# stefanch/sGDML

Measured on AMD Instinct MI355X. Metric: kernel-matrix build+solve wall-clock, N_train=1000 21-atom (aspirin-sized), lower is better.
Workload: dtype f64

## Files before the change

### include/gdml_hip.h

```cpp
#ifndef GDML_HIP_H
#define GDML_HIP_H

#include <stdint.h>

#ifdef __cplusplus
extern "C" {
#endif

typedef struct gdml_ctx gdml_ctx;

typedef enum {
  GDML_OK = 0,
  GDML_ERR_INVALID = -1,
  GDML_ERR_HIP = -2,
  GDML_ERR_OOM = -3,
  GDML_ERR_STATE = -4,
  GDML_ERR_NOT_PD = -5,
  GDML_ERR_UNSUPPORTED = -6,
  GDML_ERR_COMM = -7
} gdml_status;


int gdml_abi_version(void);

// ... 36 lines not shown
                    int64_t col_b, const int64_t* idx, int64_t n_idx, int64_t alloc_extra_rows,
                    double* K_host_out, int64_t ldk);

int gdml_assemble_A(gdml_ctx* ctx, double sig, double lam, int use_E_cstr, int64_t alloc_extra_rows);

int gdml_K_shape(gdml_ctx* ctx, int64_t* n_rows, int64_t* n_cols, int64_t* extra_rows);

int gdml_chol_set_rhs(gdml_ctx* ctx, const double* y, int64_t n);
int gdml_lu_solve(gdml_ctx* ctx, double lam, const double* y, int64_t n, double* alphas_out, int* info);
int gdml_chol_factor(gdml_ctx* ctx, double lam, int* info);
int gdml_chol_solve(gdml_ctx* ctx, const double* y, int64_t n, int n_refine, double* alphas_out);

int gdml_predict_upload_model(gdml_ctx* ctx, const double* R_desc, const double* R_d_desc_alpha,
                              int64_t M, int N, const int64_t* tril_perms, int P, double sig,
                              const double* alphas_E);
int gdml_set_alphas(gdml_ctx* ctx, const double* alphas_F, const double* alphas_E);
int gdml_predict(gdml_ctx* ctx, const double* R, int64_t B, const double* lat,
                 const double* lat_inv, double* E_out, double* F_out);

int gdml_predict_dev(gdml_ctx* ctx, const double* R_dev, int64_t B, const double* lat,
                     const double* lat_inv, double* E_dev, double* F_dev);

int gdml_predict_hessian(gdml_ctx* ctx, const double* R, int64_t B, const double* lat, const double* lat_inv,
                         double* E_out, double* F_out, double* H_out);
int gdml_predict_hessian_dev(gdml_ctx* ctx, const double* R_dev, int64_t B, const double* lat,
                             const double* lat_inv, double* E_dev, double* F_dev, double* H_dev);

int gdml_uncert_prepare(gdml_ctx* ctx, double sig, double lam, int* info);
int gdml_uncert_release(gdml_ctx* ctx);
int gdml_uncert_cross(gdml_ctx* ctx, const double* R, int64_t B, const double* lat, const double* lat_inv,
                      double* Kx_out, double* kqq_out);
int gdml_predict_cov(gdml_ctx* ctx, const double* R, int64_t B, const double* lat, const double* lat_inv, int full,
                     double* cov_out);
int gdml_predict_cov_dev(gdml_ctx* ctx, const double* R_dev, int64_t B, const double* lat, const double* lat_inv,
                         int full, double* cov_dev);

int gdml_loo(gdml_ctx* ctx, const double* alphas, int64_t n, int cov_mode, double* resid_out, double* cov_out,
             double* logdet_out, int* info);

int gdml_factor_extend(gdml_ctx* ctx, const double* R_desc_new, const double* R_d_desc_new, int64_t b, int* info);

int gdml_factor_remove(gdml_ctx* ctx, const int64_t* idx, int64_t b, int* info);

int gdml_predict_errors(gdml_ctx* ctx, const double* R, int64_t B, const double* lat,
                        const double* lat_inv, double std, double c, const double* E_ref,
                        const double* F_ref, double* sums8_out);

int gdml_kernel_matvec(gdml_ctx* ctx, double lam, int use_E_cstr, const double* v, int64_t n,
                       double* out);

typedef int (*gdml_pcg_cb)(int64_t iter, double resid, void* user);
int gdml_nystroem_factor(gdml_ctx* ctx, double lam, const int64_t* idx, int64_t m,
                         double* lev_scores_out, double* LinvKmn_host_out, int* info);
int gdml_nystroem_lev_scores(gdml_ctx* ctx, double* lev_scores_out);
int gdml_precon_apply(gdml_ctx* ctx, double lam, const double* v, int64_t n, double* out);
int gdml_pcg(gdml_ctx* ctx, double lam, int use_E_cstr, const double* y, const double* x0,
             int64_t n, double rtol, int64_t maxiter, int use_precon, gdml_pcg_cb cb,
             int64_t cb_every, void* user, double* x_out, int64_t* iters_out, double* resid_out,
             int* info_out);
int gdml_pcg_x(gdml_ctx* ctx, double* x_host_out);

int gdml_comm_unique_id(void* id128_out);
int gdml_comm_init(gdml_ctx* ctx, const void* id128, int rank, int world);
int gdml_comm_info(gdml_ctx* ctx, int* rank_out, int* world_out);
int gdml_comm_suspend(gdml_ctx* ctx, int suspend);

int gdml_dist_chol_solve(gdml_ctx* ctx, double sig, double lam, const double* y, int64_t n, double* alphas_out,
                         int* info);

typedef int (*gdml_host_allreduce)(double* buf, int64_t count, void* user);
typedef int (*gdml_host_allgather)(double* buf, int64_t chunk, void* user);
int gdml_comm_init_host(gdml_ctx* ctx, int rank, int world, gdml_host_allreduce allreduce,
                        gdml_host_allgather allgather, void* user);

int gdml_comm_stats(gdml_ctx* ctx, int64_t* calls_out, double* bytes_out);

int gdml_dev_alloc(gdml_ctx* ctx, int64_t bytes, void** dev_out);
int gdml_dev_free(gdml_ctx* ctx, void* dev);
int gdml_memcpy_h2d(gdml_ctx* ctx, void* dev, const void* host, int64_t bytes);
int gdml_memcpy_d2h(gdml_ctx* ctx, void* host, const void* dev, int64_t bytes);

int gdml_K_dev(gdml_ctx* ctx, double** K_dev_out, int64_t* ld_out);

#ifdef __cplusplus
}
#endif
#endif
```

### sgdml_amd/_lib.py

```python
import ctypes as C
import os

import numpy as np

_HERE = os.path.dirname(os.path.abspath(__file__))
LIB_PATH = os.environ.get('GDML_HIP_LIB', os.path.join(_HERE, 'libgdml_hip.so'))

GDML_OK = 0
ERR_INVALID, ERR_HIP, ERR_OOM, ERR_STATE, ERR_NOT_PD, ERR_UNSUPPORTED, ERR_COMM = -1, -2, -3, -4, -5, -6, -7
COLS_ALL, COLS_POINTS, COLS_INDEX = 0, 1, 2

_dp = C.POINTER(C.c_double)
_ip = C.POINTER(C.c_int64)
_vp = C.c_void_p
PCG_CB = C.CFUNCTYPE(C.c_int, C.c_int64, C.c_double, _vp)
HOST_COLL_CB = C.CFUNCTYPE(C.c_int, _dp, C.c_int64, _vp)

SIGNATURES = {
    'gdml_abi_version': (C.c_int, []),
    'gdml_device_count': (C.c_int, [C.POINTER(C.c_int)]),
    'gdml_device_pci_bus_id': (C.c_int, [C.c_int, C.c_char_p, C.c_int]),
    'gdml_ctx_create': (C.c_int, [C.c_int, C.POINTER(_vp)]),
    'gdml_ctx_destroy': (C.c_int, [_vp]),
    'gdml_last_error': (C.c_char_p, [_vp]),
    'gdml_sync': (C.c_int, [_vp]),
    'gdml_mem_info': (C.c_int, [_vp, _ip, _ip, _ip]),
    'gdml_mem_reserve': (C.c_int, [_vp, C.c_int64, _ip]),
    'gdml_phase_ms': (C.c_int, [_vp, C.c_char_p, _dp, _ip]),
    'gdml_profile': (C.c_int, [_vp, C.c_int]),
    'gdml_kernel_stat': (C.c_int, [_vp, C.c_char_p, _dp, _ip, _dp]),
    'gdml_desc_from_R': (C.c_int, [_vp, _vp, C.c_int64, C.c_int, _vp, _vp, _vp, _vp]),
    'gdml_sym_eig_absv': (C.c_int, [_vp, _vp, C.c_int64, C.c_int, _vp]),
    'gdml_perm_match': (C.c_int, [_vp, _vp, _vp, _vp, C.c_int64, C.c_int, _vp, _vp, _vp, C.c_int64, C.POINTER(C.c_int64)]),
    'gdml_train_upload': (C.c_int, [_vp, _vp, _vp, C.c_int64, C.c_int, _vp, C.c_int]),
    'gdml_assemble_K': (C.c_int, [_vp, C.c_double, C.c_int, C.c_int, C.c_int64, C.c_int64, _vp, C.c_int64,
                                  C.c_int64, _vp, C.c_int64]),
    'gdml_assemble_A': (C.c_int, [_vp, C.c_double, C.c_double, C.c_int, C.c_int64]),
    'gdml_K_shape': (C.c_int, [_vp, _ip, _ip, _ip]),
    'gdml_chol_set_rhs': (C.c_int, [_vp, _vp, C.c_int64]),
    'gdml_chol_factor': (C.c_int, [_vp, C.c_double, C.POINTER(C.c_int)]),
    'gdml_lu_solve': (C.c_int, [_vp, C.c_double, _vp, C.c_int64, _vp, C.POINTER(C.c_int)]),
    'gdml_chol_solve': (C.c_int, [_vp, _vp, C.c_int64, C.c_int, _vp]),
    'gdml_predict_upload_model': (C.c_int, [_vp, _vp, _vp, C.c_int64, C.c_int, _vp, C.c_int, C.c_double, _vp]),
    'gdml_set_alphas': (C.c_int, [_vp, _vp, _vp]),
    'gdml_predict': (C.c_int, [_vp, _vp, C.c_int64, _vp, _vp, _vp, _vp]),
    'gdml_predict_dev': (C.c_int, [_vp, _vp, C.c_int64, _vp, _vp, _vp, _vp]),
    'gdml_predict_hessian': (C.c_int, [_vp, _vp, C.c_int64, _vp, _vp, _vp, _vp, _vp]),
    'gdml_predict_hessian_dev': (C.c_int, [_vp, _vp, C.c_int64, _vp, _vp, _vp, _vp, _vp]),
    'gdml_uncert_prepare': (C.c_int, [_vp, C.c_double, C.c_double, C.POINTER(C.c_int)]),
    'gdml_uncert_release': (C.c_int, [_vp]),
    'gdml_uncert_cross': (C.c_int, [_vp, _vp, C.c_int64, _vp, _vp, _vp, _vp]),
    'gdml_predict_cov': (C.c_int, [_vp, _vp, C.c_int64, _vp, _vp, C.c_int, _vp]),
    'gdml_predict_cov_dev': (C.c_int, [_vp, _vp, C.c_int64, _vp, _vp, C.c_int, _vp]),
    'gdml_loo': (C.c_int, [_vp, _vp, C.c_int64, C.c_int, _vp, _vp, C.POINTER(C.c_double), C.POINTER(C.c_int)]),
    'gdml_factor_extend': (C.c_int, [_vp, _vp, _vp, C.c_int64, C.POINTER(C.c_int)]),
    'gdml_factor_remove': (C.c_int, [_vp, _vp, C.c_int64, C.POINTER(C.c_int)]),
    'gdml_kernel_matvec': (C.c_int, [_vp, C.c_double, C.c_int, _vp, C.c_int64, _vp]),
    'gdml_predict_errors': (C.c_int, [_vp, _vp, C.c_int64, _vp, _vp, C.c_double, C.c_double, _vp, _vp, _vp]),
    'gdml_nystroem_factor': (C.c_int, [_vp, C.c_double, _vp, C.c_int64, _vp, _vp, C.POINTER(C.c_int)]),
    'gdml_nystroem_lev_scores': (C.c_int, [_vp, _vp]),
    'gdml_precon_apply': (C.c_int, [_vp, C.c_double, _vp, C.c_int64, _vp]),
    'gdml_pcg': (C.c_int, [_vp, C.c_double, C.c_int, _vp, _vp, C.c_int64, C.c_double, C.c_int64, C.c_int,
                           PCG_CB, C.c_int64, _vp, _vp, _ip, _dp, C.POINTER(C.c_int)]),
    'gdml_pcg_x': (C.c_int, [_vp, _vp]),
    'gdml_dist_chol_solve': (C.c_int, [_vp, C.c_double, C.c_double, _vp, C.c_int64, _vp, C.POINTER(C.c_int)]),
    'gdml_comm_unique_id': (C.c_int, [_vp]),
    'gdml_comm_init': (C.c_int, [_vp, _vp, C.c_int, C.c_int]),
    'gdml_comm_info': (C.c_int, [_vp, C.POINTER(C.c_int), C.POINTER(C.c_int)]),
    'gdml_comm_suspend': (C.c_int, [_vp, C.c_int]),
    'gdml_comm_init_host': (C.c_int, [_vp, C.c_int, C.c_int, HOST_COLL_CB, HOST_COLL_CB, _vp]),
    'gdml_comm_stats': (C.c_int, [_vp, _ip, _dp]),
    'gdml_set_option': (C.c_int, [_vp, C.c_char_p, C.c_double]),
    'gdml_get_option': (C.c_int, [_vp, C.c_char_p, _dp, C.POINTER(C.c_int)]),
    'gdml_dev_alloc': (C.c_int, [_vp, C.c_int64, C.POINTER(_vp)]),
    'gdml_dev_free': (C.c_int, [_vp, _vp]),
    'gdml_memcpy_h2d': (C.c_int, [_vp, _vp, _vp, C.c_int64]),
    'gdml_memcpy_d2h': (C.c_int, [_vp, _vp, _vp, C.c_int64]),
    'gdml_K_dev': (C.c_int, [_vp, C.POINTER(_vp), _ip]),
}

_lib = None


class GDMLHipError(RuntimeError):
    pass


def load():
    global _lib
    if _lib is not None:
        return _lib
    if not os.path.exists(LIB_PATH):
        raise ImportError(
            'libgdml_hip.so not found at {} -- build it with `python -c "import __graft_entry__ as g; '
            'g.build()"` or `make -C sgdml_amd/csrc`. There is no CPU fallback.'.format(LIB_PATH)
        )
    lib = C.CDLL(LIB_PATH)
    for name, (res, args) in SIGNATURES.items():
        fn = getattr(lib, name)
        fn.restype = res
        fn.argtypes = args
    _lib = lib
    return lib


def device_count():
    n = C.c_int(0)
    load().gdml_device_count(C.byref(n))
    return n.value


def device_pci_bus_id(device):
    buf = C.create_string_buffer(64)
    if load().gdml_device_pci_bus_id(int(device), buf, 64) != 0:
        return None
    return buf.value.decode() or None


def preflight(attempts=3, timeout=180):
    import subprocess
    import sys

    if device_count() < 1:
        return 0
    code = ('import numpy as np; from sgdml_amd import _lib; c = _lib.Context(0); '
            'c.desc_from_R(np.arange(18.0).reshape(2, 9) ** 1.5, 3); c.close()')
    root = os.path.dirname(os.path.dirname(os.path.abspath(__file__)))
    err = ''
    for k in range(1, attempts + 1):
        try:
            p = subprocess.run([sys.executable, '-c', code], cwd=root, capture_output=True, text=True, timeout=timeout)
            if p.returncode == 0:
                return k
            err = (p.stderr or '')[-400:]
        except subprocess.TimeoutExpired:
            err = 'timeout'
    raise RuntimeError('GPU preflight failed %d times: %s' % (attempts, err))


def _ptr(a):
    return None if a is None else a.ctypes.data_as(_vp)


def f64(a):
    return None if a is None else np.ascontiguousarray(a, dtype=np.float64)


def i64(a):
    return None if a is None else np.ascontiguousarray(a, dtype=np.int64)


def _digest(a):
    try:
        import xxhash

        return xxhash.xxh64(memoryview(a).cast('B')).hexdigest()
    except ImportError:
        import hashlib

        return hashlib.md5(memoryview(a).cast('B')).hexdigest()

# ... 519 lines not shown
```

### sgdml_amd/csrc/chol.hip

```cpp
#include "common.h"
#include <type_traits>
#include <utility>

typedef double d4 __attribute__((ext_vector_type(4)));
typedef double d2 __attribute__((ext_vector_type(2)));

#define GT 128
#define GBK 16
#define GPITCH 17

struct GemmArgs {
  const double* A;
  const double* B;
  double* C;
  int64_t M, N, K, lda, ldb, ldc;
  int lower;
  int tiles_m, tiles_n;
  int64_t n_super;
  int64_t s_begin;
  int super_n;
  int aligned;
  int cyc_W, cyc_rank;
  int64_t cyc_lb0, cyc_nb, cyc_col0, cyc_block_rows;
  double* diagA;
  int diag_nbw;
  int64_t diag_off;
  int* diag_info;
  int col0_first;
  int* ready;
  int ready_target, ready_rows;
  const double* A2;
  const double* B2;
  double* C2;
  int64_t M2, N2, K2;
  int tiles2;
};

__global__ void __launch_bounds__(256, 2) gemm_nt_sub_diag_kernel(GemmArgs g);

template <bool FULL>
__device__ __forceinline__ void gemm_load_tile(const double* __restrict__ G, int64_t ld,
                                               int64_t row0, int64_t nrows, int64_t k0, int64_t K,
                                               int tid, d2 (&r)[4]) {
#pragma unroll
  for (int s = 0; s < 4; ++s) {
    int cidx = tid + 256 * s;
    int row = cidx >> 3, kc = (cidx & 7) * 2;
    int64_t gr = row0 + row, gk = k0 + kc;
    if (FULL) {
      r[s] = *reinterpret_cast<const d2*>(G + gr * ld + gk);
    } else {
      int64_t cr = gr < nrows ? gr : nrows - 1;
      int64_t ck0 = gk < K ? gk : K - 1, ck1 = gk + 1 < K ? gk + 1 : K - 1;
      double v0 = G[cr * ld + ck0], v1 = G[cr * ld + ck1];
      d2 v;
      v.x = (gr < nrows && gk < K) ? v0 : 0.0;
      v.y = (gr < nrows && gk + 1 < K) ? v1 : 0.0;
      r[s] = v;
    }
  }
}

__device__ __forceinline__ void gemm_load_tile_g(const double* __restrict__ base, const unsigned (&off)[4], d2 (&r)[4]) {
  typedef const __attribute__((address_space(1))) char* gcptr;
  typedef const __attribute__((address_space(1))) d2* gd2ptr;
  const uint64_t p = reinterpret_cast<uint64_t>(base);
  const uint32_t lo = __builtin_amdgcn_readfirstlane((uint32_t)p), hi = __builtin_amdgcn_readfirstlane((uint32_t)(p >> 32));
  gcptr b = (gcptr)(((uint64_t)hi << 32) | lo);
#pragma unroll
  for (int s = 0; s < 4; ++s) r[s] = *(gd2ptr)(b + off[s]);
}

__device__ __forceinline__ void gemm_store_tile16(double* __restrict__ S, int tid, const d2 (&r)[4]) {
  d2* S2 = reinterpret_cast<d2*>(S);
#pragma unroll
  for (int s = 0; s < 4; ++s) {
    const int cidx = tid + 256 * s;
    const int row = cidx >> 3, kq = cidx & 7;
    S2[kq * 128 + (row ^ kq)] = r[s];
  }
}

template <bool FULL, bool OW>
__device__ __forceinline__ void gemm_tile_body(const GemmArgs& g, double (*lds)[2][GT * GPITCH], int64_t row0, int64_t col0) {
  const int tid = threadIdx.x, lane = tid & 63, wave = tid >> 6;
  const int wm = wave >> 1, wn = wave & 1;
  const int li = lane & 15, lk = lane >> 4;

  const int wu = __builtin_amdgcn_readfirstlane(wave);
  double* const Ct = g.C + (row0 + (wu >> 1) * 64) * g.ldc + col0 + (wu & 1) * 64;
  const unsigned coff = (unsigned)lk * (unsigned)g.ldc + (unsigned)li;
  d4 acc[4][4];
#pragma unroll
  for (int i = 0; i < 4; ++i)
#pragma unroll
    for (int j = 0; j < 4; ++j) {
      if (FULL && !OW) {
#pragma unroll
        for (int r = 0; r < 4; ++r) acc[i][j][r] = -(Ct + (int64_t)(i * 16 + 4 * r) * g.ldc)[coff + j * 16];
      } else {
        acc[i][j] = (d4){0.0, 0.0, 0.0, 0.0};
      }
    }

  const int nk32 = (int)((g.K + GBK - 1) / GBK);
  d2 ra[4], rb[4];
  gemm_load_tile<FULL>(g.A, g.lda, row0, g.M, 0, g.K, tid, ra);
  gemm_load_tile<FULL>(g.B, g.ldb, col0, g.N, 0, g.K, tid, rb);
  gemm_store_tile16(lds[0][0], tid, ra);
  gemm_store_tile16(lds[0][1], tid, rb);
  __syncthreads();

  const int c16 = lane & 15, gq = lane >> 4;
  unsigned offA[4], offB[4];
#pragma unroll
  for (int s4 = 0; s4 < 4; ++s4) {
    const int cidx = tid + 256 * s4;
    offA[s4] = (unsigned)(((int64_t)(cidx >> 3) * g.lda + (cidx & 7) * 2) * 8);
    offB[s4] = (unsigned)(((int64_t)(cidx >> 3) * g.ldb + (cidx & 7) * 2) * 8);
  }
  const double* const Abase = g.A + row0 * g.lda;
// ... 52 lines not shown
  };
  for (int kt = 0; kt + 1 < nk32; ++kt) step(kt, std::true_type{});
  step(nk32 - 1, std::false_type{});

  if (FULL) {
    double* Ct2g = Ct;
    unsigned coff2 = coff;
    asm volatile("" : "+v"(Ct2g), "+v"(coff2));
    __attribute__((address_space(1))) double* Ct2 = (__attribute__((address_space(1))) double*)Ct2g;
#pragma unroll
    for (int j = 0; j < 4; ++j)
#pragma unroll
      for (int i = 0; i < 4; ++i)
#pragma unroll
        for (int r = 0; r < 4; ++r) (Ct2 + (int64_t)(i * 16 + 4 * r) * g.ldc)[coff2 + j * 16] = -acc[i][j][r];
    return;
  }
  if constexpr (OW) {
#pragma unroll
    for (int j = 0; j < 4; ++j) {
      const int64_t gc = col0 + wn * 64 + j * 16 + li;
#pragma unroll
      for (int i = 0; i < 4; ++i)
#pragma unroll
        for (int r = 0; r < 4; ++r) {
          const int64_t gr = row0 + wm * 64 + i * 16 + lk + 4 * r;
          if (gc < g.N && gr < g.M) g.C[gr * g.ldc + gc] = -acc[i][j][r];
        }
    }
    return;
  }
#pragma unroll
  for (int j = 0; j < 4; ++j) {
    double cv[4][4];
    const int64_t gc = col0 + wn * 64 + j * 16 + li;
    const bool cok = gc < g.N;
#pragma unroll
    for (int i = 0; i < 4; ++i)
#pragma unroll
      for (int r = 0; r < 4; ++r) {
        const int64_t gr = row0 + wm * 64 + i * 16 + lk + 4 * r;
        const int64_t cr = gr < g.M ? gr : g.M - 1, cc = cok ? gc : g.N - 1;
        cv[i][r] = g.C[cr * g.ldc + cc];
      }
#pragma unroll
    for (int i = 0; i < 4; ++i)
#pragma unroll
      for (int r = 0; r < 4; ++r) {
        const int64_t gr = row0 + wm * 64 + i * 16 + lk + 4 * r;
        if (cok && gr < g.M) g.C[gr * g.ldc + gc] = cv[i][r] - acc[i][j][r];
      }
  }
}

template <bool OW>
__device__ __forceinline__ void gemm_block(const GemmArgs& g, double (*lds)[2][GT * GPITCH], int64_t b) {
  if (b < g.tiles2) {
    const int tn2 = (int)((g.N2 + GT - 1) / GT);
    const int64_t ti = b / tn2, tj = b - ti * tn2;
    if (ti < tn2 && tj > ti) return;
    GemmArgs h = g;
    h.A = g.A2; h.B = g.B2; h.C = g.C2; h.M = g.M2; h.N = g.N2; h.K = g.K2;
    h.aligned = ((reinterpret_cast<uintptr_t>(g.A2) | reinterpret_cast<uintptr_t>(g.B2)) & 15) == 0 && g.aligned;
    const int64_t row0 = ti * GT, col0 = tj * GT;
    const bool full = (row0 + GT <= h.M) && (col0 + GT <= h.N) && ((h.K & (GBK - 1)) == 0) && h.aligned;
    if (full)
      gemm_tile_body<true, false>(h, lds, row0, col0);
    else
      gemm_tile_body<false, false>(h, lds, row0, col0);
    if (g.ready && ti < g.ready_rows && tj < g.ready_rows) {
      __threadfence();
      __syncthreads();
      if (threadIdx.x == 0) atomicAdd(g.ready, 1);
    }
    return;
  }
  b -= g.tiles2;
  const int64_t xcd = b & 7, loc = b >> 3;
  const int64_t s = g.s_begin + (loc >> 6) * 8 + xcd;
  const int within = (int)(loc & 63);
  if (s >= g.n_super) return;
  int64_t SI, SJ;
  if (g.lower) {
    int64_t sr = s, shift = 0;
    const int64_t sm = (g.tiles_m + 7) / 8;
    if (g.col0_first) {
      if (s < sm) { SI = s; SJ = 0; sr = -1; }
      else { sr = s - sm; shift = 1; }
    }
    if (sr >= 0) {
      SI = (int64_t)((sqrt(8.0 * (double)sr + 1.0) - 1.0) * 0.5);
      while (SI * (SI + 1) / 2 > sr) --SI;
      while ((SI + 1) * (SI + 2) / 2 <= sr) ++SI;
      SJ = sr - SI * (SI + 1) / 2;
      SI += shift; SJ += shift;
    }
  } else {
    SI = s / g.super_n;
    SJ = s - SI * g.super_n;
  }
  const int64_t ti = SI * 8 + (within >> 3), tj = SJ * 8 + (within & 7);
  if (ti >= g.tiles_m || tj >= g.tiles_n) return;
  if (g.lower && tj > ti) return;
  const int64_t row0 = ti * GT, col0 = tj * GT;
  if (g.cyc_W > 0 && row0 + GT <= g.cyc_block_rows) {
    const int64_t gb = (g.cyc_lb0 + row0 / g.cyc_nb) * g.cyc_W + g.cyc_rank;
    const int64_t grow_last = gb * g.cyc_nb + (row0 + GT - 1) % g.cyc_nb;
    if (g.cyc_col0 + col0 > grow_last) return;
  }
  const bool full = (row0 + GT <= g.M) && (col0 + GT <= g.N) && ((g.K & (GBK - 1)) == 0) && g.aligned;
  if (full)
    gemm_tile_body<true, OW>(g, lds, row0, col0);
  else
    gemm_tile_body<false, OW>(g, lds, row0, col0);
  if (g.ready && g.tiles2 == 0 && ti < g.ready_rows && tj < g.ready_rows) {
    __threadfence();
    __syncthreads();
    if (threadIdx.x == 0) atomicAdd(g.ready, 1);
  }
}

__global__ void __launch_bounds__(256, 2) gemm_nt_sub_kernel(GemmArgs g) {
  __shared__ __attribute__((aligned(16))) double lds[2][2][GT * GPITCH];
  gemm_block<false>(g, lds, blockIdx.x);
}


__global__ void __launch_bounds__(256, 2) gemm_nt_neg_kernel(GemmArgs g) {
  __shared__ __attribute__((aligned(16))) double lds[2][2][GT * GPITCH];
  gemm_block<true>(g, lds, blockIdx.x);
}

struct DiagJob {
  double* A = nullptr;
  int nbw = 0;
  int64_t off = 0;
  int* ready = nullptr;
  int ready_target = 0;
  bool col0_first = false;
  const double* A2 = nullptr;
  const double* B2 = nullptr;
  double* C2 = nullptr;
  int64_t M2 = 0, N2 = 0, K2 = 0;
};

static int launch_gemm_nt_sub_part(gdml_ctx* ctx, hipStream_t st, const double* A, int64_t lda,
                                   const double* B, int64_t ldb, double* C, int64_t ldc, int64_t M,
                                   int64_t N, int64_t K, int lower, double f0, double f1, bool timed,
                                   const DiagJob* diag = nullptr, const CyclicLower* cyc = nullptr, bool overwrite = false) {
  if (M <= 0 || N <= 0 || K <= 0) return GDML_OK;
  GemmArgs g;
  g.A = A; g.B = B; g.C = C; g.M = M; g.N = N; g.K = K; g.lda = lda; g.ldb = ldb; g.ldc = ldc;
  g.lower = lower;
  g.diagA = nullptr; g.diag_nbw = 0; g.diag_off = 0; g.diag_info = nullptr;
  g.cyc_W = 0; g.cyc_rank = 0; g.cyc_lb0 = 0; g.cyc_nb = 0; g.cyc_col0 = 0; g.cyc_block_rows = 0;
  g.col0_first = (diag && diag->col0_first) ? 1 : 0;
  g.ready = nullptr; g.ready_target = 0; g.ready_rows = 0;
  g.A2 = g.B2 = nullptr; g.C2 = nullptr; g.M2 = g.N2 = g.K2 = 0; g.tiles2 = 0;
  if (cyc) { g.cyc_W = cyc->W; g.cyc_rank = cyc->rank; g.cyc_lb0 = cyc->lb0; g.cyc_nb = cyc->nb; g.cyc_col0 = cyc->col0; g.cyc_block_rows = cyc->block_rows; }
  g.aligned = ((reinterpret_cast<uintptr_t>(A) | reinterpret_cast<uintptr_t>(B)) & 15) == 0 &&
              (lda % 2 == 0) && (ldb % 2 == 0);
  g.tiles_m = (int)((M + GT - 1) / GT);
  g.tiles_n = (int)((N + GT - 1) / GT);
  int64_t sm = (g.tiles_m + 7) / 8, sn = (g.tiles_n + 7) / 8;
  g.super_n = (int)sn;
  const int64_t n_super_all = lower ? sm * (sm + 1) / 2 : sm * sn;
  g.s_begin = (int64_t)(f0 * (double)n_super_all);
  g.n_super = (f1 >= 1.0) ? n_super_all : (int64_t)(f1 * (double)n_super_all);
  const bool has_diag = diag && diag->A;
  if (g.n_super <= g.s_begin) {
    if (!has_diag) return GDML_OK;
    g.n_super = g.s_begin;
  }
  int64_t groups = (g.n_super - g.s_begin + 7) / 8;
  int64_t blocks = groups * 512;
  const int slot = (timed && st == (ctx->kt_stream ? ctx->kt_stream : ctx->stream)) ? ktime_begin(ctx) : -1;
  if (has_diag) {
    g.diagA = diag->A; g.diag_nbw = diag->nbw; g.diag_off = diag->off; g.diag_info = ctx->d_info;
    if (diag->ready) { g.ready = diag->ready; g.ready_target = diag->ready_target; g.ready_rows = diag->nbw * 64 / GT; }
    if (diag->A2 && diag->M2 > 0) {
      g.A2 = diag->A2; g.B2 = diag->B2; g.C2 = diag->C2; g.M2 = diag->M2; g.N2 = diag->N2; g.K2 = diag->K2;
      g.tiles2 = (int)(ceil_div(g.M2, GT) * ceil_div(g.N2, GT));
    }
    hipLaunchKernelGGL(gemm_nt_sub_diag_kernel, dim3((unsigned)(blocks + 1 + g.tiles2)), dim3(256), 0, st, g);
  } else if (overwrite)
    hipLaunchKernelGGL(gemm_nt_neg_kernel, dim3((unsigned)blocks), dim3(256), 0, st, g);
  else
    hipLaunchKernelGGL(gemm_nt_sub_kernel, dim3((unsigned)blocks), dim3(256), 0, st, g);
  const double part = (double)(g.n_super - g.s_begin) / (double)n_super_all;
  ktime_end(ctx, slot, has_diag ? "gemm_nt_sub_diag" : "gemm_nt_sub",
            part * (lower ? (double)M * (double)(M + 1) * (double)K : 2.0 * (double)M * (double)N * (double)K) +
                2.0 * (double)g.M2 * (double)g.N2 * (double)g.K2);
  ctx->launch_counter++;
  HIP_CHECK(ctx, hipGetLastError());
  return GDML_OK;
}

int launch_gemm_nt_sub(gdml_ctx* ctx, hipStream_t st, const double* A, int64_t lda,
                              const double* B, int64_t ldb, double* C, int64_t ldc, int64_t M,
                              int64_t N, int64_t K, int lower) {
  return launch_gemm_nt_sub_part(ctx, st, A, lda, B, ldb, C, ldc, M, N, K, lower, 0.0, 1.0, true);
}

int launch_gemm_nt_neg(gdml_ctx* ctx, hipStream_t st, const double* A, int64_t lda, const double* B, int64_t ldb,
                       double* C, int64_t ldc, int64_t M, int64_t N, int64_t K) {
  return launch_gemm_nt_sub_part(ctx, st, A, lda, B, ldb, C, ldc, M, N, K, 0, 0.0, 1.0, true, nullptr, nullptr, true);
}

int launch_gemm_nt_sub_cyclic(gdml_ctx* ctx, hipStream_t st, const double* A, int64_t lda, const double* B, int64_t ldb,
                              double* C, int64_t ldc, int64_t M, int64_t N, int64_t K, const CyclicLower& cyc) {
  return launch_gemm_nt_sub_part(ctx, st, A, lda, B, ldb, C, ldc, M, N, K, 0, 0.0, 1.0, true, nullptr, &cyc);
}

__device__ __forceinline__ double readlane_f64(double v, int l) {
  const int lo = __builtin_amdgcn_readlane(__double2loint(v), l);
  const int hi = __builtin_amdgcn_readlane(__double2hiint(v), l);
  return __hiloint2double(hi, lo);
}
__device__ __forceinline__ int potrf64_wave(double* T, double* cb , int lane) {
  double row[64];
#pragma unroll
  for (int c = 0; c < 64; ++c) row[c] = T[lane * 65 + c];
  int fail = 0;
#pragma unroll
  for (int jb = 0; jb < 8; ++jb) {
#pragma unroll
    for (int jj = 0; jj < 8; ++jj) {
      const int j = 8 * jb + jj;
      const double d = readlane_f64(row[j], j);
      if (!(d > 0.0) && fail == 0) fail = j + 1;
      double ri = __builtin_amdgcn_rsq(d);
      ri = ri * (1.5 - 0.5 * d * ri * ri);
      ri = ri * (1.5 - 0.5 * d * ri * ri);
      const double lr = row[j] * ri;
      row[j] = lr;
#pragma unroll
      for (int c = j + 1; c < 8 * jb + 8; ++c) row[c] -= lr * readlane_f64(lr, c);
    }
    if (jb < 7) {
// ... 638 lines not shown
        for (int j = 0; j < 2; ++j)
          acc[i][j] = __builtin_amdgcn_mfma_f64_16x16x4f64(-a[i][ch][sidx], bb[j][ch][sidx], acc[i][j], 0, 0, 0);
#pragma unroll
  for (int i = 0; i < 2; ++i)
#pragma unroll
    for (int j = 0; j < 2; ++j)
#pragma unroll
      for (int r = 0; r < 4; ++r)
        if (crow[i][r] < m && ccol[j] < ncols) C[(int64_t)crow[i][r] * ld + ccol[j]] = acc[i][j][r];
}

int panel_factor_steps(gdml_ctx* ctx, hipStream_t st, double* A, int64_t n, int64_t ld, int64_t k0, int64_t nb);

static int panel_factor(gdml_ctx* ctx, hipStream_t st, double* A, int64_t n, int64_t ld, int64_t k0,
                        int64_t nb) {
  const int64_t below = n - k0 - nb;
  const bool aligned = (reinterpret_cast<uintptr_t>(A) & 31) == 0 && (ld % 4 == 0) && (k0 % 4 == 0);
  if (nb % 64 == 0 && nb <= 512 && below > 0 && aligned) {
    GDML_TRY(panel_factor_steps(ctx, st, A, k0 + nb, ld, k0, nb));
    return launch_panel_trsm(ctx, st, A + k0 * ld + k0, A + (k0 + nb) * ld + k0, ld, (int)nb, below);
  }
  return panel_factor_steps(ctx, st, A, n, ld, k0, nb);
}

int panel_factor_steps(gdml_ctx* ctx, hipStream_t st, double* A, int64_t n, int64_t ld, int64_t k0,
                       int64_t nb) {
  double* save = nullptr;
  GDML_TRY(ctx_slot(ctx, SLOT_PANEL_SAVE, 2 * 4096 * 8, &save));
  const double* Lprev = nullptr;
  double* Aprev = nullptr;
  int wprev = 0, flip = 0;
  for (int64_t jj = 0; jj < nb; jj += 64) {
    const int64_t c0 = k0 + jj;
    const int w = (int)((nb - jj < 64) ? nb - jj : 64);
    double* Ad = A + c0 * ld + c0;
    const int64_t m = n - c0 - w;
    if (m > 0) {
      double* X = A + (c0 + w) * ld + c0;
      double* Lsave = save + flip * 4096;
      hipLaunchKernelGGL(potrf_trsm64_kernel, dim3((unsigned)ceil_div(m, 256)), dim3(256), 0, st, Ad, X, ld, w, m,
                         c0, ctx->d_info, Lsave, Lprev, Aprev, wprev);
      ctx->launch_counter++;
      Lprev = Lsave;
      Aprev = Ad;
      wprev = w;
      flip ^= 1;
      const int64_t ncols = k0 + nb - (c0 + w);
      if (ncols > 0) {
        const bool al32 = (reinterpret_cast<uintptr_t>(X) & 31) == 0 && (ld % 4 == 0);
        if (w == 64 && m <= 2048 && al32) {
          const int tiles = (int)(ceil_div(m, 32) * ceil_div(ncols, 32));
          hipLaunchKernelGGL(rank64_update_kernel, dim3((unsigned)ceil_div(tiles, 4)), dim3(256), 0, st, X, X,
                             A + (c0 + w) * ld + (c0 + w), ld, (int)m, (int)ncols, 1);
          ctx->launch_counter++;
        } else {
          GDML_TRY(launch_gemm_nt_sub(ctx, st, X, ld, X, ld, A + (c0 + w) * ld + (c0 + w), ld, m, ncols, w, 0));
        }
      }
    } else {
      if (Lprev) {
        hipLaunchKernelGGL(writeback_block_kernel, dim3(1), dim3(256), 0, st, Lprev, Aprev, ld, wprev);
        ctx->launch_counter++;
        Lprev = nullptr;
      }
      hipLaunchKernelGGL(potrf64_kernel, dim3(1), dim3(64), 0, st, Ad, ld, w, c0, ctx->d_info);
      ctx->launch_counter++;
    }
  }
  if (Lprev) {
    hipLaunchKernelGGL(writeback_block_kernel, dim3(1), dim3(256), 0, st, Lprev, Aprev, ld, wprev);
    ctx->launch_counter++;
  }
  return GDML_OK;
}

int chol_factor_device(gdml_ctx* ctx, double* A, int64_t n, int64_t ld, int* info_out, int64_t n_rows) {
  if (n_rows < n) n_rows = n;
  HIP_CHECK(ctx, hipMemsetAsync(ctx->d_info, 0, sizeof(int), ctx->stream));
  int64_t NB = (int64_t)ctx_opt(ctx, "chol.nb", 512);
  if (NB < 64 || NB % 64 || NB > 512) NB = 512;
  hipStream_t st = ctx->stream;
  const int64_t min_rows = (int64_t)ctx_opt(ctx, "chol.fused_min_rows", 12288);
  int64_t OB = (int64_t)ctx_opt(ctx, "chol.outer", 1024);
  if (OB != 2 * NB || NB % GT != 0) OB = NB;
  const int64_t outer_min_rows = (int64_t)ctx_opt(ctx, "chol.outer_min_rows", 16384);
  auto width_at = [&](int64_t c0) -> int64_t {
    const int64_t left = n - (c0 + OB);
    const int64_t w = (OB > NB && left > 0 && left >= outer_min_rows) ? OB : NB;
    return (n - c0 < w) ? n - c0 : w;
  };
  int64_t k0 = 0, nb = (n < NB) ? n : NB;
  int ready_count = 0;
  HIP_CHECK(ctx, hipMemsetAsync(ctx->d_info + 6, 0, 2 * sizeof(int), ctx->stream));
  GDML_TRY(panel_factor(ctx, st, A, n_rows, ld, 0, nb));
  for (;;) {
    const int64_t t0 = k0 + nb;
    if (t0 >= n) break;
    const int64_t nb2 = width_at(t0);
    const int64_t t1 = t0 + nb2;
    const double* P = A + t0 * ld + k0;
    const bool fuse = (nb2 % 64 == 0) && (n - t1 >= min_rows) && (n_rows - t1 > 0);
    if (fuse && nb2 == 2 * NB) {
      const int64_t ta = t0 + NB;
      const int64_t sm = (ceil_div(n_rows - t0, GT) + 7) / 8, n_super_all = sm * (sm + 1) / 2;
      int64_t s_split = n_super_all / 2;
      if (s_split < sm) s_split = sm;
      const double fs = ((double)s_split + 0.5) / (double)n_super_all;
      DiagJob dj;
      dj.A = A + t0 * ld + t0; dj.nbw = (int)(NB / 64); dj.off = t0;
      dj.col0_first = true;
      dj.ready = ctx->d_info + 6;
      const int block_tiles = (int)((NB / GT) * (NB / GT + 1) / 2);
      ready_count += block_tiles;
      dj.ready_target = ready_count;
      GDML_TRY(launch_gemm_nt_sub_part(ctx, st, P, ld, P, ld, A + t0 * ld + t0, ld, n_rows - t0, n - t0, nb, 1, 0.0, fs, true,
                                       &dj));
      double* Xa = A + ta * ld + t0;
      GDML_TRY(launch_panel_trsm(ctx, st, A + t0 * ld + t0, Xa, ld, (int)NB, n_rows - ta));
      dj.A = A + ta * ld + ta; dj.off = ta;
      dj.A2 = Xa; dj.B2 = Xa; dj.C2 = A + ta * ld + ta; dj.M2 = n_rows - ta; dj.N2 = NB; dj.K2 = NB;
      ready_count += block_tiles;
      dj.ready_target = ready_count;
      GDML_TRY(launch_gemm_nt_sub_part(ctx, st, P, ld, P, ld, A + t0 * ld + t0, ld, n_rows - t0, n - t0, nb, 1, fs, 1.0, true,
                                       &dj));
      GDML_TRY(launch_panel_trsm(ctx, st, A + ta * ld + ta, A + t1 * ld + ta, ld, (int)NB, n_rows - t1));
    } else {
      GDML_TRY(launch_gemm_nt_sub(ctx, st, P, ld, P, ld, A + t0 * ld + t0, ld, n_rows - t0, nb2, nb, 0));
      const double* P1 = A + t1 * ld + k0;
      if (fuse) {
        DiagJob dj;
        dj.A = A + t0 * ld + t0;
        dj.nbw = (int)(nb2 / 64);
        dj.off = t0;
        GDML_TRY(launch_gemm_nt_sub_part(ctx, st, P1, ld, P1, ld, A + t1 * ld + t1, ld, n_rows - t1, n - t1, nb, 1, 0.0,
                                         1.0, true, &dj));
        GDML_TRY(launch_panel_trsm(ctx, st, A + t0 * ld + t0, A + t1 * ld + t0, ld, (int)nb2, n_rows - t1));
      } else if (t1 < n) {
        hipStream_t sp = ctx->stream2;
        HIP_CHECK(ctx, hipEventRecord(ctx->ev_la[0], st));
        HIP_CHECK(ctx, hipStreamWaitEvent(sp, ctx->ev_la[0], 0));
        GDML_TRY(panel_factor(ctx, sp, A, n_rows, ld, t0, nb2));
        HIP_CHECK(ctx, hipEventRecord(ctx->ev_la[1], sp));
        GDML_TRY(launch_gemm_nt_sub(ctx, st, P1, ld, P1, ld, A + t1 * ld + t1, ld, n_rows - t1, n - t1, nb, 1));
        HIP_CHECK(ctx, hipStreamWaitEvent(st, ctx->ev_la[1], 0));
      } else {
        GDML_TRY(panel_factor(ctx, st, A, n_rows, ld, t0, nb2));
      }
    }
    k0 = t0;
    nb = nb2;
  }
  HIP_CHECK(ctx, hipGetLastError());
  int info8[8] = {0};
  HIP_CHECK(ctx, hipMemcpyAsync(info8, ctx->d_info, sizeof(info8), hipMemcpyDeviceToHost, ctx->stream));
  HIP_CHECK(ctx, hipStreamSynchronize(ctx->stream));
  if (info8[7] != 0)
    return gdml_fail(ctx, GDML_ERR_HIP, "Cholesky: the diagonal-block workgroup gave up waiting for its tiles (schedule bug)");
  if (info_out) *info_out = info8[0];
  return GDML_OK;
}

template <bool TRANS>
__device__ __forceinline__ double tri_solve64_wave(const double* Ls, double b, int lane) {
  double v[64];
#pragma unroll
  for (int k = 0; k < 64; ++k) v[k] = TRANS ? Ls[k * 65 + lane] : Ls[lane * 65 + k];
  double sol = 0.0;
  if (!TRANS) {
#pragma unroll
    for (int c = 0; c < 64; ++c) {
      const double t = b / v[c];
      const double zc = __shfl(t, c, 64);
      if (lane == c) sol = zc;
      b -= v[c] * zc;
    }
  } else {
#pragma unroll
    for (int r = 63; r >= 0; --r) {
      const double t = b / v[r];
      const double xr = __shfl(t, r, 64);
      if (lane == r) sol = xr;
      b -= v[r] * xr;
    }
  }
  return sol;
}

__device__ __forceinline__ void load_block64(const double* __restrict__ L, int64_t ld, int64_t c0,
                                             int w, double* Ls, int tid, int T) {
  for (int e = tid; e < 64 * 64; e += T) {
    int r = e >> 6, c = e & 63;
    double v = (r == c) ? 1.0 : 0.0;
    if (r < w && c < w && c <= r) v = L[(c0 + r) * ld + c0 + c];
    Ls[r * 65 + c] = v;
  }
}

__global__ void __launch_bounds__(256) trsv_fwd_kernel(const double* __restrict__ L, int64_t ld,
                                                       int64_t n, int64_t c0, int w,
                                                       double* __restrict__ b,
                                                       double* __restrict__ z_out) {
  __shared__ __attribute__((aligned(16))) double Ls[64 * 65];
  __shared__ double z[64];
  const int tid = threadIdx.x, lane = tid & 63, wave = tid >> 6;
  load_block64(L, ld, c0, w, Ls, tid, 256);
  __syncthreads();
  if (wave == 0) {
    const double bi = lane < w ? b[c0 + lane] : 0.0;
    const double zi = tri_solve64_wave<false>(Ls, bi, lane);
    z[lane] = zi;
    if (blockIdx.x == 0 && lane < w) z_out[c0 + lane] = zi;
  }
  __syncthreads();
  const int64_t first = c0 + w;
  const double zl = lane < w ? z[lane] : 0.0;
  for (int64_t r = first + (int64_t)blockIdx.x * 4 + wave; r < n; r += (int64_t)gridDim.x * 4) {
    double v = lane < w ? L[r * ld + c0 + lane] * zl : 0.0;
    v = wave_sum(v);
    if (lane == 0) b[r] -= v;
  }
}

__global__ void __launch_bounds__(256) trsv_bwd_kernel(const double* __restrict__ L, int64_t ld,
                                                       int64_t c0, int w, double* __restrict__ b,
                                                       double* __restrict__ x_out) {
  __shared__ __attribute__((aligned(16))) double Ls[64 * 65];
  __shared__ double x[64];
  const int tid = threadIdx.x, lane = tid & 63, wave = tid >> 6;
  load_block64(L, ld, c0, w, Ls, tid, 256);
  __syncthreads();
  if (wave == 0) {
    const double bi = lane < w ? b[c0 + lane] : 0.0;
    const double xi = tri_solve64_wave<true>(Ls, bi, lane);
    x[lane] = xi;
    if (blockIdx.x == 0 && lane < w) x_out[c0 + lane] = xi;
  }
  __syncthreads();
  for (int64_t c = (int64_t)blockIdx.x * 256 + tid; c < c0; c += (int64_t)gridDim.x * 256) {
    double s = 0.0;
    for (int r = 0; r < w; ++r) s += L[(c0 + r) * ld + c] * x[r];
    b[c] -= s;
// ... 246 lines not shown
```

### sgdml_amd/csrc/ctx.hip

```cpp
#include <stdarg.h>

#include <mutex>

#include "common.h"

static std::string g_create_err;

int gdml_fail(gdml_ctx* ctx, int code, const char* fmt, ...) {
  char buf[1024];
  va_list ap;
  va_start(ap, fmt);
  vsnprintf(buf, sizeof(buf), fmt, ap);
  va_end(ap);
  if (ctx)
    ctx->err = buf;
  else
    g_create_err = buf;
  return code;
}

extern "C" int gdml_abi_version(void) { return 4; }

static const char* kKnownOptions[] = {
    "asm.wave", "asm.j_chunk", "asm.lower", "asm.strip", "asm.i_chunk",
    "asm.pts", "asm.pts_nv", "asm.pts_nt", "asm.pts_xcd", "asm.pts_i_chunk", "asm.pts_debug", "asm.perm_debug", "asm.perm_w", "asm.perm_lds_kb", "asm.perm_level", "asm.perm_nimg", "asm.perm_pg", "asm.perm_na", "asm.perm_fast_store", "asm.perm_i_chunk", "asm.perm_compact", "asm.perm_lds_rows", "asm.big1", "asm.perm2", "asm.perm2_min_n", "asm.perm2_min_p", "asm.perm2_split", "asm.perm2_post", "asm.perm2_ed", "asm.perm2_es", "asm.perm2_direct", "asm.perm2_chunk", "asm.perm2_i_chunk", "asm.perm2_debug",
    "nys.trsm_left", "nys.syrk_split", "predict.wide_pad", "predict.tn_fill", "chol.nb", "pcg.gemv_plain",
    "chol.fused_min_rows", "chol.outer", "chol.outer_min_rows", "trsm.debug",
    "trsv.persist", "predict.wave_only", "predict.mfma", "predict.fill", "predict.mfma_wide", "predict.fused", "predict.fused_rows", "predict.fused_spin",
    "lu.nb", "comm.force_collectives", "nys.force_qr", "nys.force_fail", "dist.nb", "dist.lookahead", "dist.force_panels", "pcg.depth", "pcg.precon_form", "pcg.f32_rows_per", "pcg.f32_rw", "pcg.f32_min_pivot", "pcg.f32_last_min_pivot", "pcg.f32_gram_rows", "pcg.f32_inplace",
    "predict.hess_generic", "predict.hess_chunk_rows", "predict.cov_chunk", "predict.cov_global", "chol.loo_chunk", "chol.extend_chunk", "chol.remove_chunk"};

double ctx_opt(const gdml_ctx* ctx, const char* key, double dflt) {
  auto it = ctx->opts.find(key);
  return it == ctx->opts.end() ? dflt : it->second;
}

extern "C" int gdml_set_option(gdml_ctx* ctx, const char* key, double value) {
  if (!ctx || !key) return GDML_ERR_INVALID;
  for (const char* k : kKnownOptions)
    if (strcmp(k, key) == 0) {
      ctx->opts[key] = value;
      return GDML_OK;
    }
  return gdml_fail(ctx, GDML_ERR_INVALID, "gdml_set_option: unknown option '%s'", key);
}

extern "C" int gdml_get_option(gdml_ctx* ctx, const char* key, double* value_out, int* is_set_out) {
  if (!ctx || !key) return GDML_ERR_INVALID;
  auto it = ctx->opts.find(key);
  if (value_out) *value_out = it == ctx->opts.end() ? 0.0 : it->second;
  if (is_set_out) *is_set_out = it != ctx->opts.end();
  return GDML_OK;
}

static void options_from_env(gdml_ctx* ctx) {
  const char* e = getenv("GDML_OPTIONS");
  if (!e) return;
  std::string s(e);
  size_t pos = 0;
  while (pos < s.size()) {
    size_t end = s.find(',', pos);
    if (end == std::string::npos) end = s.size();
    const std::string kv = s.substr(pos, end - pos);
    const size_t eq = kv.find('=');
    if (eq != std::string::npos) (void)gdml_set_option(ctx, kv.substr(0, eq).c_str(), atof(kv.c_str() + eq + 1));
    pos = end + 1;
  }
}

struct ArenaBlock {
  int64_t off, bytes;
  gdml_ctx* owner;
};
struct DeviceArena {
  void* base = nullptr;
  int64_t bytes = 0;
  std::vector<ArenaBlock> blocks;
};
static DeviceArena g_arena[64];
static std::mutex g_arena_mu;
static const int64_t kArenaMinRequest = (int64_t)1 << 30;
static const int64_t kArenaAlign = (int64_t)2 << 20;

static DeviceArena* arena_of(const gdml_ctx* ctx) { return (ctx->device >= 0 && ctx->device < 64) ? &g_arena[ctx->device] : nullptr; }

static void* arena_carve(DeviceArena* a, gdml_ctx* ctx, int64_t bytes) {
  const int64_t need = (bytes + kArenaAlign - 1) / kArenaAlign * kArenaAlign;
  int64_t off = 0;
  size_t pos = 0;
  for (; pos <= a->blocks.size(); ++pos) {
    const int64_t end = pos < a->blocks.size() ? a->blocks[pos].off : a->bytes;
    if (end - off >= need) break;
    if (pos < a->blocks.size()) off = a->blocks[pos].off + a->blocks[pos].bytes;
  }
  if (pos > a->blocks.size()) return nullptr;
  a->blocks.insert(a->blocks.begin() + (long)pos, ArenaBlock{off, need, ctx});
  return (char*)a->base + off;
}
static bool arena_owns(const DeviceArena* a, const void* p) {
  return a && a->base && (const char*)p >= (const char*)a->base && (const char*)p < (const char*)a->base + a->bytes;
}
static void arena_release(DeviceArena* a, const void* p) {
  const int64_t off = (const char*)p - (const char*)a->base;
  for (size_t i = 0; i < a->blocks.size(); ++i)
    if (a->blocks[i].off == off) {
      a->blocks.erase(a->blocks.begin() + (long)i);
      return;
    }
}
static void arena_release_owner(gdml_ctx* ctx) {
// ... 400 lines not shown
```

Baseline: 1.284.

## Generalize fused Cholesky outer step to multiple inner diagonal blocks

Replaces the hard-coded two-block fused outer step of the blocked Cholesky with a loop over m = OB/NB inner diagonal blocks, allowing an outer width of 4*NB. The tile scheduler now orders the first q super-tile columns ahead of the rest, and launch ranges are split into m parts. Each part's diagonal workgroup factors its block once its tiles are ready. The aim is fewer trailing-update passes over the large matrix and more overlap of panel work with the update. The risk is changed tile ordering and sync targets on the default path, plus extra launches per step.

```diff
diff --git a/include/gdml_hip.h b/include/gdml_hip.h
--- a/include/gdml_hip.h
+++ b/include/gdml_hip.h
@@ -142,6 +142,8 @@
 
 int gdml_K_dev(gdml_ctx* ctx, double** K_dev_out, int64_t* ld_out);
 
+int gdml_chol_tile_order(int64_t sm, int q, int m, int64_t* si_out, int64_t* sj_out, int64_t* begin_out);
+
 #ifdef __cplusplus
 }
 #endif
diff --git a/sgdml_amd/_lib.py b/sgdml_amd/_lib.py
--- a/sgdml_amd/_lib.py
+++ b/sgdml_amd/_lib.py
@@ -77,6 +77,7 @@
     'gdml_memcpy_h2d': (C.c_int, [_vp, _vp, _vp, C.c_int64]),
     'gdml_memcpy_d2h': (C.c_int, [_vp, _vp, _vp, C.c_int64]),
     'gdml_K_dev': (C.c_int, [_vp, C.POINTER(_vp), _ip]),
+    'gdml_chol_tile_order': (C.c_int, [C.c_int64, C.c_int, C.c_int, _ip, _ip, _ip]),
 }
 
 _lib = None
diff --git a/sgdml_amd/csrc/chol.hip b/sgdml_amd/csrc/chol.hip
--- a/sgdml_amd/csrc/chol.hip
+++ b/sgdml_amd/csrc/chol.hip
@@ -26,7 +26,7 @@
   int diag_nbw;
   int64_t diag_off;
   int* diag_info;
-  int col0_first;
+  int lead_cols;
   int* ready;
   int ready_target, ready_rows;
   const double* A2;
@@ -37,6 +37,28 @@
 };
 
 __global__ void __launch_bounds__(256, 2) gemm_nt_sub_diag_kernel(GemmArgs g);
+
+__host__ __device__ __forceinline__ void lower_super_tile(int64_t sm, int q, int64_t s, int64_t& SI, int64_t& SJ) {
+  for (int c = 0; c < q; ++c) {
+    if (s < sm - c) { SI = c + s; SJ = c; return; }
+    s -= sm - c;
+  }
+  SI = (int64_t)((sqrt(8.0 * (double)s + 1.0) - 1.0) * 0.5);
+  while (SI * (SI + 1) / 2 > s) --SI;
+  while ((SI + 1) * (SI + 2) / 2 <= s) ++SI;
+  SJ = s - SI * (SI + 1) / 2;
+  SI += q; SJ += q;
+}
+
+static int64_t lower_launch_begin(int64_t sm, int q, int m, int i) {
+  const int64_t n_all = sm * (sm + 1) / 2;
+  if (i <= 0) return 0;
+  if (i >= m) return n_all;
+  int64_t s1 = n_all / m, lead = 0;
+  for (int c = 0; c < q; ++c) lead += sm - c;
+  if (s1 < lead) s1 = lead;
+  return s1 + (n_all - s1) * (i - 1) / (m - 1);
+}
 
 template <bool FULL>
 __device__ __forceinline__ void gemm_load_tile(const double* __restrict__ G, int64_t ld,
@@ -255,19 +277,7 @@
   if (s >= g.n_super) return;
   int64_t SI, SJ;
   if (g.lower) {
-    int64_t sr = s, shift = 0;
-    const int64_t sm = (g.tiles_m + 7) / 8;
-    if (g.col0_first) {
-      if (s < sm) { SI = s; SJ = 0; sr = -1; }
-      else { sr = s - sm; shift = 1; }
-    }
-    if (sr >= 0) {
-      SI = (int64_t)((sqrt(8.0 * (double)sr + 1.0) - 1.0) * 0.5);
-      while (SI * (SI + 1) / 2 > sr) --SI;
-      while ((SI + 1) * (SI + 2) / 2 <= sr) ++SI;
-      SJ = sr - SI * (SI + 1) / 2;
-      SI += shift; SJ += shift;
-    }
+    lower_super_tile((g.tiles_m + 7) / 8, g.lead_cols, s, SI, SJ);
   } else {
     SI = s / g.super_n;
     SJ = s - SI * g.super_n;
@@ -310,7 +320,7 @@
   int64_t off = 0;
   int* ready = nullptr;
   int ready_target = 0;
-  bool col0_first = false;
+  int lead_cols = 0;
   const double* A2 = nullptr;
   const double* B2 = nullptr;
   double* C2 = nullptr;
@@ -327,7 +337,7 @@
   g.lower = lower;
   g.diagA = nullptr; g.diag_nbw = 0; g.diag_off = 0; g.diag_info = nullptr;
   g.cyc_W = 0; g.cyc_rank = 0; g.cyc_lb0 = 0; g.cyc_nb = 0; g.cyc_col0 = 0; g.cyc_block_rows = 0;
-  g.col0_first = (diag && diag->col0_first) ? 1 : 0;
+  g.lead_cols = diag ? diag->lead_cols : 0;
   g.ready = nullptr; g.ready_target = 0; g.ready_rows = 0;
   g.A2 = g.B2 = nullptr; g.C2 = nullptr; g.M2 = g.N2 = g.K2 = 0; g.tiles2 = 0;
   if (cyc) { g.cyc_W = cyc->W; g.cyc_rank = cyc->rank; g.cyc_lb0 = cyc->lb0; g.cyc_nb = cyc->nb; g.cyc_col0 = cyc->col0; g.cyc_block_rows = cyc->block_rows; }
@@ -1132,11 +1142,15 @@
   hipStream_t st = ctx->stream;
   const int64_t min_rows = (int64_t)ctx_opt(ctx, "chol.fused_min_rows", 12288);
   int64_t OB = (int64_t)ctx_opt(ctx, "chol.outer", 1024);
-  if (OB != 2 * NB || NB % GT != 0) OB = NB;
+  if ((OB != 2 * NB && OB != 4 * NB) || NB % GT != 0) OB = NB;
   const int64_t outer_min_rows = (int64_t)ctx_opt(ctx, "chol.outer_min_rows", 16384);
+  const int64_t outer4_min_rows = (int64_t)ctx_opt(ctx, "chol.outer4_min_rows", 16384);
   auto width_at = [&](int64_t c0) -> int64_t {
-    const int64_t left = n - (c0 + OB);
-    const int64_t w = (OB > NB && left > 0 && left >= outer_min_rows) ? OB : NB;
+    int64_t w = NB;
+    for (int64_t m = OB / NB; m > 1; m /= 2) {
+      const int64_t left = n - (c0 + m * NB);
+      if (left > 0 && left >= (m == 4 ? outer4_min_rows : outer_min_rows)) { w = m * NB; break; }
+    }
     return (n - c0 < w) ? n - c0 : w;
   };
   int64_t k0 = 0, nb = (n < NB) ? n : NB;
@@ -1150,30 +1164,30 @@
     const int64_t t1 = t0 + nb2;
     const double* P = A + t0 * ld + k0;
     const bool fuse = (nb2 % 64 == 0) && (n - t1 >= min_rows) && (n_rows - t1 > 0);
-    if (fuse && nb2 == 2 * NB) {
-      const int64_t ta = t0 + NB;
+    if (fuse && nb2 > NB) {
+      const int m = (int)(nb2 / NB);
       const int64_t sm = (ceil_div(n_rows - t0, GT) + 7) / 8, n_super_all = sm * (sm + 1) / 2;
-      int64_t s_split = n_super_all / 2;
-      if (s_split < sm) s_split = sm;
-      const double fs = ((double)s_split + 0.5) / (double)n_super_all;
+      const int q = (int)ceil_div(nb2, 8 * GT);
       DiagJob dj;
-      dj.A = A + t0 * ld + t0; dj.nbw = (int)(NB / 64); dj.off = t0;
-      dj.col0_first = true;
+      dj.nbw = (int)(NB / 64);
+      dj.lead_cols = q;
       dj.ready = ctx->d_info + 6;
       const int block_tiles = (int)((NB / GT) * (NB / GT + 1) / 2);
-      ready_count += block_tiles;
-      dj.ready_target = ready_count;
-      GDML_TRY(launch_gemm_nt_sub_part(ctx, st, P, ld, P, ld, A + t0 * ld + t0, ld, n_rows - t0, n - t0, nb, 1, 0.0, fs, true,
-                                       &dj));
-      double* Xa = A + ta * ld + t0;
-      GDML_TRY(launch_panel_trsm(ctx, st, A + t0 * ld + t0, Xa, ld, (int)NB, n_rows - ta));
-      dj.A = A + ta * ld + ta; dj.off = ta;
-      dj.A2 = Xa; dj.B2 = Xa; dj.C2 = A + ta * ld + ta; dj.M2 = n_rows - ta; dj.N2 = NB; dj.K2 = NB;
-      ready_count += block_tiles;
-      dj.ready_target = ready_count;
-      GDML_TRY(launch_gemm_nt_sub_part(ctx, st, P, ld, P, ld, A + t0 * ld + t0, ld, n_rows - t0, n - t0, nb, 1, fs, 1.0, true,
-                                       &dj));
-      GDML_TRY(launch_panel_trsm(ctx, st, A + ta * ld + ta, A + t1 * ld + ta, ld, (int)NB, n_rows - t1));
+      for (int i = 0; i < m; ++i) {
+        const int64_t ti = t0 + i * NB;
+        double* D = A + ti * ld + ti;
+        dj.A = D; dj.off = ti;
+        if (i > 0) {
+          dj.A2 = A + ti * ld + t0; dj.B2 = dj.A2; dj.C2 = D; dj.M2 = n_rows - ti; dj.N2 = NB; dj.K2 = i * NB;
+        }
+        ready_count += block_tiles;
+        dj.ready_target = ready_count;
+        const double f0 = (i == 0) ? 0.0 : ((double)lower_launch_begin(sm, q, m, i) + 0.5) / (double)n_super_all;
+        const double f1 = (i == m - 1) ? 1.0 : ((double)lower_launch_begin(sm, q, m, i + 1) + 0.5) / (double)n_super_all;
+        GDML_TRY(launch_gemm_nt_sub_part(ctx, st, P, ld, P, ld, A + t0 * ld + t0, ld, n_rows - t0, n - t0, nb, 1, f0, f1, true,
+                                         &dj));
+        GDML_TRY(launch_panel_trsm(ctx, st, D, D + NB * ld, ld, (int)NB, n_rows - (ti + NB)));
+      }
     } else {
       GDML_TRY(launch_gemm_nt_sub(ctx, st, P, ld, P, ld, A + t0 * ld + t0, ld, n_rows - t0, nb2, nb, 0));
       const double* P1 = A + t1 * ld + k0;
@@ -1207,6 +1221,13 @@
   if (info8[7] != 0)
     return gdml_fail(ctx, GDML_ERR_HIP, "Cholesky: the diagonal-block workgroup gave up waiting for its tiles (schedule bug)");
   if (info_out) *info_out = info8[0];
+  return GDML_OK;
+}
+
+extern "C" int gdml_chol_tile_order(int64_t sm, int q, int m, int64_t* si_out, int64_t* sj_out, int64_t* begin_out) {
+  if (sm < 1 || q < 0 || q > sm || m < 1 || !si_out || !sj_out || !begin_out) return GDML_ERR_INVALID;
+  for (int64_t s = 0; s < sm * (sm + 1) / 2; ++s) lower_super_tile(sm, q, s, si_out[s], sj_out[s]);
+  for (int i = 0; i <= m; ++i) begin_out[i] = lower_launch_begin(sm, q, m, i);
   return GDML_OK;
 }
 
diff --git a/sgdml_amd/csrc/ctx.hip b/sgdml_amd/csrc/ctx.hip
--- a/sgdml_amd/csrc/ctx.hip
+++ b/sgdml_amd/csrc/ctx.hip
@@ -25,7 +25,7 @@
     "asm.wave", "asm.j_chunk", "asm.lower", "asm.strip", "asm.i_chunk",
     "asm.pts", "asm.pts_nv", "asm.pts_nt", "asm.pts_xcd", "asm.pts_i_chunk", "asm.pts_debug", "asm.perm_debug", "asm.perm_w", "asm.perm_lds_kb", "asm.perm_level", "asm.perm_nimg", "asm.perm_pg", "asm.perm_na", "asm.perm_fast_store", "asm.perm_i_chunk", "asm.perm_compact", "asm.perm_lds_rows", "asm.big1", "asm.perm2", "asm.perm2_min_n", "asm.perm2_min_p", "asm.perm2_split", "asm.perm2_post", "asm.perm2_ed", "asm.perm2_es", "asm.perm2_direct", "asm.perm2_chunk", "asm.perm2_i_chunk", "asm.perm2_debug",
     "nys.trsm_left", "nys.syrk_split", "predict.wide_pad", "predict.tn_fill", "chol.nb", "pcg.gemv_plain",
-    "chol.fused_min_rows", "chol.outer", "chol.outer_min_rows", "trsm.debug",
+    "chol.fused_min_rows", "chol.outer", "chol.outer_min_rows", "chol.outer4_min_rows", "trsm.debug",
     "trsv.persist", "predict.wave_only", "predict.mfma", "predict.fill", "predict.mfma_wide", "predict.fused", "predict.fused_rows", "predict.fused_spin",
     "lu.nb", "comm.force_collectives", "nys.force_qr", "nys.force_fail", "dist.nb", "dist.lookahead", "dist.force_panels", "pcg.depth", "pcg.precon_form", "pcg.f32_rows_per", "pcg.f32_rw", "pcg.f32_min_pivot", "pcg.f32_last_min_pivot", "pcg.f32_gram_rows", "pcg.f32_inplace",
     "predict.hess_generic", "predict.hess_chunk_rows", "predict.cov_chunk", "predict.cov_global", "chol.loo_chunk", "chol.extend_chunk", "chol.remove_chunk"};
```

Measured after the change: 1.285. No clear change (+0.1%).
